# andrewjong/SwapNet

Hardware: NVIDIA H100
Metric: images/sec (G+D fwd+bwd) warp-stage 512x512 (higher is better)
Workload: dtype fp16/bf16-split x3 tensor-core products, fp32 accumulate (fp32-faithful)

## Files before the change

### swapnet_b200/csrc/common.cuh

```cuda
#pragma once
#include <cuda_runtime.h>
#include <cuda.h>
#include <cuda_bf16.h>
#include <cuda_fp16.h>
#include <stdint.h>
#include <stdio.h>
#include <string.h>

void sn_set_error(const char* fmt, ...);
#define SN_OK 0
#define SN_ERR_INVALID (-1)
#define SN_ERR_CUDA (-2)
#define SN_ERR_UNSUPPORTED (-3)
#define SN_NUM_SMS 132
#ifndef SN_FMT_BF16
#define SN_FMT_BF16 0
#define SN_FMT_F16 1
#endif

#define SN_CHECK_CUDA(expr)                                                        \
  do {                                                                             \
    cudaError_t _e = (expr);                                                       \
    if (_e != cudaSuccess) {                                                       \
      sn_set_error("%s:%d CUDA error %s: %s", __FILE__, __LINE__, #expr,           \
// ... 80 lines not shown
      "cp.async.bulk.tensor.3d.shared::cluster.global.mbarrier::complete_tx::bytes"
      " [%0], [%1, {%3, %4, %5}], [%2];"
      :
      : "r"(smem_u32(dst)), "l"(reinterpret_cast<uint64_t>(desc)), "r"(smem_u32(bar)), "r"(c0), "r"(c1), "r"(c2)
      : "memory");
}
__device__ __forceinline__ void tma_load_5d(const void* desc, uint64_t* bar, void* dst, int c0,
                                            int c1, int c2, int c3, int c4) {
  asm volatile(
      "cp.async.bulk.tensor.5d.shared::cluster.global.mbarrier::complete_tx::bytes"
      " [%0], [%1, {%3, %4, %5, %6, %7}], [%2];"
      :
      : "r"(smem_u32(dst)), "l"(reinterpret_cast<uint64_t>(desc)), "r"(smem_u32(bar)), "r"(c0),
        "r"(c1), "r"(c2), "r"(c3), "r"(c4)
      : "memory");
}

__device__ __forceinline__ void wgmma_fence() { asm volatile("wgmma.fence.sync.aligned;" ::: "memory"); }
__device__ __forceinline__ void wgmma_commit() { asm volatile("wgmma.commit_group.sync.aligned;" ::: "memory"); }
template <int N>
__device__ __forceinline__ void wgmma_wait() {
  asm volatile("wgmma.wait_group.sync.aligned %0;" ::"n"(N) : "memory");
}
template <int R>
__device__ __forceinline__ void wgmma_fence_acc(float (&d)[R]) {
#pragma unroll
  for (int i = 0; i < R; ++i) asm volatile("" : "+f"(d[i])::"memory");
}

template <int N, bool F16>
struct Wgmma;
template <> struct Wgmma<16, false> {
  template <int TA, int TB>
  static __device__ __forceinline__ void mma(float (&d)[8], uint64_t a, uint64_t b, int scale_d) {
    asm volatile(
        "{\n.reg .pred p;\nsetp.ne.b32 p, %10, 0;\n"
        "wgmma.mma_async.sync.aligned.m64n16k16.f32.bf16.bf16 "
        "{%0, %1, %2, %3, %4, %5, %6, %7}, %8, %9, p, 1, 1, %11, %12;\n}\n"
        : "+f"(d[0]), "+f"(d[1]), "+f"(d[2]), "+f"(d[3]), "+f"(d[4]), "+f"(d[5]), "+f"(d[6]), "+f"(d[7])
        : "l"(a), "l"(b), "r"(scale_d), "n"(TA), "n"(TB));
  }
};
template <> struct Wgmma<16, true> {
  template <int TA, int TB>
  static __device__ __forceinline__ void mma(float (&d)[8], uint64_t a, uint64_t b, int scale_d) {
    asm volatile(
// ... 72 lines not shown
};
template <> struct Wgmma<128, false> {
  template <int TA, int TB>
  static __device__ __forceinline__ void mma(float (&d)[64], uint64_t a, uint64_t b, int scale_d) {
    asm volatile(
        "{\n.reg .pred p;\nsetp.ne.b32 p, %66, 0;\n"
        "wgmma.mma_async.sync.aligned.m64n128k16.f32.bf16.bf16 "
        "{%0, %1, %2, %3, %4, %5, %6, %7, %8, %9, %10, %11, %12, %13, %14, %15, %16, %17, %18, %19, %20, %21, %22, %23, %24, %25, %26, %27, %28, %29, %30, %31, %32, %33, %34, %35, %36, %37, %38, %39, %40, %41, %42, %43, %44, %45, %46, %47, %48, %49, %50, %51, %52, %53, %54, %55, %56, %57, %58, %59, %60, %61, %62, %63}, %64, %65, p, 1, 1, %67, %68;\n}\n"
        : "+f"(d[0]), "+f"(d[1]), "+f"(d[2]), "+f"(d[3]), "+f"(d[4]), "+f"(d[5]), "+f"(d[6]), "+f"(d[7]), "+f"(d[8]), "+f"(d[9]), "+f"(d[10]), "+f"(d[11]), "+f"(d[12]), "+f"(d[13]), "+f"(d[14]), "+f"(d[15]), "+f"(d[16]), "+f"(d[17]), "+f"(d[18]), "+f"(d[19]), "+f"(d[20]), "+f"(d[21]), "+f"(d[22]), "+f"(d[23]), "+f"(d[24]), "+f"(d[25]), "+f"(d[26]), "+f"(d[27]), "+f"(d[28]), "+f"(d[29]), "+f"(d[30]), "+f"(d[31]), "+f"(d[32]), "+f"(d[33]), "+f"(d[34]), "+f"(d[35]), "+f"(d[36]), "+f"(d[37]), "+f"(d[38]), "+f"(d[39]), "+f"(d[40]), "+f"(d[41]), "+f"(d[42]), "+f"(d[43]), "+f"(d[44]), "+f"(d[45]), "+f"(d[46]), "+f"(d[47]), "+f"(d[48]), "+f"(d[49]), "+f"(d[50]), "+f"(d[51]), "+f"(d[52]), "+f"(d[53]), "+f"(d[54]), "+f"(d[55]), "+f"(d[56]), "+f"(d[57]), "+f"(d[58]), "+f"(d[59]), "+f"(d[60]), "+f"(d[61]), "+f"(d[62]), "+f"(d[63])
        : "l"(a), "l"(b), "r"(scale_d), "n"(TA), "n"(TB));
  }
};
template <> struct Wgmma<128, true> {
  template <int TA, int TB>
  static __device__ __forceinline__ void mma(float (&d)[64], uint64_t a, uint64_t b, int scale_d) {
    asm volatile(
        "{\n.reg .pred p;\nsetp.ne.b32 p, %66, 0;\n"
        "wgmma.mma_async.sync.aligned.m64n128k16.f32.f16.f16 "
        "{%0, %1, %2, %3, %4, %5, %6, %7, %8, %9, %10, %11, %12, %13, %14, %15, %16, %17, %18, %19, %20, %21, %22, %23, %24, %25, %26, %27, %28, %29, %30, %31, %32, %33, %34, %35, %36, %37, %38, %39, %40, %41, %42, %43, %44, %45, %46, %47, %48, %49, %50, %51, %52, %53, %54, %55, %56, %57, %58, %59, %60, %61, %62, %63}, %64, %65, p, 1, 1, %67, %68;\n}\n"
        : "+f"(d[0]), "+f"(d[1]), "+f"(d[2]), "+f"(d[3]), "+f"(d[4]), "+f"(d[5]), "+f"(d[6]), "+f"(d[7]), "+f"(d[8]), "+f"(d[9]), "+f"(d[10]), "+f"(d[11]), "+f"(d[12]), "+f"(d[13]), "+f"(d[14]), "+f"(d[15]), "+f"(d[16]), "+f"(d[17]), "+f"(d[18]), "+f"(d[19]), "+f"(d[20]), "+f"(d[21]), "+f"(d[22]), "+f"(d[23]), "+f"(d[24]), "+f"(d[25]), "+f"(d[26]), "+f"(d[27]), "+f"(d[28]), "+f"(d[29]), "+f"(d[30]), "+f"(d[31]), "+f"(d[32]), "+f"(d[33]), "+f"(d[34]), "+f"(d[35]), "+f"(d[36]), "+f"(d[37]), "+f"(d[38]), "+f"(d[39]), "+f"(d[40]), "+f"(d[41]), "+f"(d[42]), "+f"(d[43]), "+f"(d[44]), "+f"(d[45]), "+f"(d[46]), "+f"(d[47]), "+f"(d[48]), "+f"(d[49]), "+f"(d[50]), "+f"(d[51]), "+f"(d[52]), "+f"(d[53]), "+f"(d[54]), "+f"(d[55]), "+f"(d[56]), "+f"(d[57]), "+f"(d[58]), "+f"(d[59]), "+f"(d[60]), "+f"(d[61]), "+f"(d[62]), "+f"(d[63])
        : "l"(a), "l"(b), "r"(scale_d), "n"(TA), "n"(TB));
  }
};


__device__ __forceinline__ uint64_t gmma_smem_desc(uint32_t smem_addr, uint32_t lbo_bytes, uint32_t sbo_bytes,
                                                   uint32_t layout = 1) {
  uint64_t d = 0;
  d |= (uint64_t)((smem_addr >> 4) & 0x3FFF);
  d |= (uint64_t)((lbo_bytes >> 4) & 0x3FFF) << 16;
  d |= (uint64_t)((sbo_bytes >> 4) & 0x3FFF) << 32;
  d |= (uint64_t)(layout & 3u) << 62;
  return d;
}
__host__ __device__ __forceinline__ uint32_t gmma_layout_of_chunk(int chunk) {
  return chunk >= 64 ? 1u : (chunk == 32 ? 2u : 3u);
}

__device__ __forceinline__ void split16(float v, int fmt, uint16_t& hi, uint16_t& lo) {
  if (fmt == SN_FMT_F16) {
    if (fabsf(v) <= 3.402823466e38f) v = fminf(fmaxf(v, -65504.f), 65504.f);
    const __half h = __float2half_rn(v);
    const __half l = __float2half_rn(v - __half2float(h));
    hi = __half_as_ushort(h);
    lo = __half_as_ushort(l);
  } else {
    const __nv_bfloat16 h = __float2bfloat16_rn(v);
// ... 17 lines not shown
```

### swapnet_b200/csrc/gemm_tc.cu

```cuda
#include "common.cuh"
#include "plan.h"

namespace {

constexpr int kBlockM = 128;
constexpr int kTileRing = 4;
constexpr int kTileBytes = 16384;
constexpr int kConsumerWarps = 8;
constexpr int kProducerWarp = kConsumerWarps;
constexpr int kThreads = (kConsumerWarps + 1) * 32;

template <int NSPLIT>
struct Cfg {
  static constexpr int kPlanes = NSPLIT == 3 ? 2 : 1;
  static constexpr int kStages = NSPLIT == 3 ? 3 : 6;
  static constexpr int kStageBytes = kPlanes * 2 * kTileBytes;
  static constexpr int kSmemBytes = kStages * kStageBytes + 1024;
};

__device__ __forceinline__ float apply_act(float v, int act) {
  if (act == SN_ACT_TANH) return tanhf(v);
  return v;
}

__device__ __forceinline__ float quad_col_sum(float v) {
  v += __shfl_xor_sync(0xffffffffu, v, 4);
  v += __shfl_xor_sync(0xffffffffu, v, 8);
  v += __shfl_xor_sync(0xffffffffu, v, 16);
  return v;
}

template <int NSPLIT, int CW, int BN, bool F16>
__global__ void __launch_bounds__(kThreads, 1)
tap_gemm_kernel(const __grid_constant__ TapGemmParams p, const int m_tiles, const int n_tiles, const int total_tiles) {
  const auto tile_coords = [&](int tile, int& mt, int& nt, int& z) {
    nt = tile % n_tiles;
    const int rest = tile / n_tiles;
    mt = rest % m_tiles;
    z = rest / m_tiles;
  };
  using C = Cfg<NSPLIT>;
  extern __shared__ uint8_t smem_raw[];
  __shared__ __align__(8) uint64_t full_bar[C::kStages];
  __shared__ __align__(8) uint64_t empty_bar[C::kStages];
  __shared__ __align__(8) uint64_t tr_full[kTileRing];
  __shared__ __align__(8) uint64_t tr_empty[kTileRing];
  __shared__ int tile_ring[kTileRing];

  const uint32_t smem_base = (smem_u32(smem_raw) + 1023u) & ~1023u;
  uint8_t* smem = smem_raw + (smem_base - smem_u32(smem_raw));
  const int warp = threadIdx.x >> 5;
  const int lane = threadIdx.x & 31;

  constexpr int cw = CW;
  constexpr int tps = 64 / cw;
  const int tpp = p.ntaps / p.nphase;
  const int k_iters = cw == 64 ? tpp * p.chunks : tpp / tps;

  if (threadIdx.x == 0) {
    for (int s = 0; s < C::kStages; ++s) {
      mbar_init(&full_bar[s], 1);
      mbar_init(&empty_bar[s], 2);
    }
    for (int r = 0; r < kTileRing; ++r) {
      mbar_init(&tr_full[r], 1);
      mbar_init(&tr_empty[r], kConsumerWarps);
    }
    mbar_fence_init();
  }
  if (warp == kProducerWarp && lane == 0) {
    for (int pl = 0; pl < C::kPlanes; ++pl) {
      tma_prefetch_desc(&p.tmA[pl]);
      tma_prefetch_desc(&p.tmB[pl]);
    }
  }
  __syncthreads();

  if (warp == kProducerWarp) {
    if (lane == 0) {
      const uint32_t stage_tx = C::kPlanes * (p.a_rows * 128 + p.block_n * 128);
      uint32_t it = 0, tcount = 0;
      for (int tile = blockIdx.x;; ++tcount) {
        const int next = tile < total_tiles ? (int)gridDim.x + atomicAdd(p.tile_counter, 1) : total_tiles;
        const uint32_t slot = tcount % kTileRing, rph = (tcount / kTileRing) & 1;
        mbar_wait(&tr_empty[slot], rph ^ 1);
        tile_ring[slot] = tile < total_tiles ? tile : -1;
        mbar_arrive(&tr_full[slot]);
        if (tile >= total_tiles) break;
        int mt, nt, z;
        tile_coords(tile, mt, nt, z);
        const int ncol0 = nt * p.block_n;
        const int tap0 = z * tpp;
        const int w0 = (mt % p.tiles_w) * p.tw;
        const int h0 = ((mt / p.tiles_w) % p.tiles_h) * p.th;
        const int n0 = (mt / (p.tiles_w * p.tiles_h)) * p.nb;
        for (int k = 0; k < k_iters; ++k, ++it) {
          const uint32_t s = it % C::kStages;
          const uint32_t ph = (it / C::kStages) & 1;
          mbar_wait(&empty_bar[s], ph ^ 1);
          mbar_expect_tx(&full_bar[s], stage_tx);
          uint8_t* st = smem + s * C::kStageBytes;
          if (cw == 64) {
            const int t = k / p.chunks;
            const int ch = k - t * p.chunks;
            const TapDesc tap = p.taps[tap0 + t];
            if (p.a_merged) {
              tma_load_5d(&p.tmA[0], &full_bar[s], st, tap.c_off + ch * 64, w0 + tap.dw, h0 + tap.dh, n0, 0);
            } else {
#pragma unroll
              for (int pl = 0; pl < C::kPlanes; ++pl)
                tma_load_5d(&p.tmA[pl], &full_bar[s], st + pl * kTileBytes, tap.c_off + ch * 64,
                            w0 + tap.dw, tap.hp, h0 + tap.dh, n0);
            }
            if (p.b_merged) {
              tma_load_3d(&p.tmB[0], &full_bar[s], st + C::kPlanes * kTileBytes, tap.kb_off + ch * 64, ncol0, 0);
            } else {
#pragma unroll
              for (int pl = 0; pl < C::kPlanes; ++pl)
                tma_load_2d(&p.tmB[pl], &full_bar[s], st + (C::kPlanes + pl) * kTileBytes,
                            tap.kb_off + ch * 64, ncol0);
            }
          } else {
            constexpr int sub = 128 * cw * 2;
#pragma unroll
            for (int j = 0; j < tps; ++j) {
              const TapDesc tap = p.taps[tap0 + k * tps + j];
#pragma unroll
              for (int pl = 0; pl < C::kPlanes; ++pl)
                tma_load_5d(&p.tmA[pl], &full_bar[s], st + pl * kTileBytes + j * sub, tap.c_off,
                            w0 + tap.dw, tap.hp, h0 + tap.dh, n0);
            }
            const int kb = p.taps[tap0 + k * tps].kb_off;
            if (p.b_merged) {
              tma_load_3d(&p.tmB[0], &full_bar[s], st + C::kPlanes * kTileBytes, kb, ncol0, 0);
            } else {
#pragma unroll
              for (int pl = 0; pl < C::kPlanes; ++pl)
                tma_load_2d(&p.tmB[pl], &full_bar[s], st + (C::kPlanes + pl) * kTileBytes, kb, ncol0);
            }
          }
        }
        tile = next;
      }
    }
  } else {
    const int wg = warp >> 2;
    const int quad = lane & 3;
    const int row0 = wg * 64 + (warp & 3) * 16 + (lane >> 2);
    int w_i[2], h_i[2], n_i[2];
#pragma unroll
    for (int h = 0; h < 2; ++h) {
      const int row = row0 + 8 * h;
      w_i[h] = row % p.tw;
      h_i[h] = (row / p.tw) % p.th;
      n_i[h] = row / (p.tw * p.th);
    }
    const float oscale = p.b_scale ? p.b_scale[1] : 1.f;
    float acc[BN / 2];
    uint32_t it = 0;
    for (uint32_t tcount = 0;; ++tcount) {
      const uint32_t slot = tcount % kTileRing, rph = (tcount / kTileRing) & 1;
      mbar_wait(&tr_full[slot], rph);
      const int tile = tile_ring[slot];
      __syncwarp();
      if (lane == 0) mbar_arrive(&tr_empty[slot]);
      if (tile < 0) break;
      for (int k = 0; k < k_iters; ++k, ++it) {
        const uint32_t s = it % C::kStages;
        const uint32_t ph = (it / C::kStages) & 1;
        mbar_wait(&full_bar[s], ph);
        const uint32_t st = smem_base + s * C::kStageBytes;
        constexpr uint32_t a_layout = cw >= 64 ? 1u : (cw == 32 ? 2u : 3u);
        constexpr uint32_t a_sbo = 8u * cw * 2u;
        const uint32_t a_row0 = (uint32_t)wg * 64u * cw * 2u;
        const uint64_t a_hi = gmma_smem_desc(st + a_row0, 16, a_sbo, a_layout);
        const uint64_t b_hi = gmma_smem_desc(st + C::kPlanes * kTileBytes, 16, 1024);
        const uint64_t a_lo = gmma_smem_desc(st + p.a_lo_off + a_row0, 16, a_sbo, a_layout);
        const uint64_t b_lo = gmma_smem_desc(st + C::kPlanes * kTileBytes + p.b_lo_off, 16, 1024);
        constexpr uint32_t sub16 = (uint32_t)(128 * cw * 2) >> 4;
        wgmma_fence();
#pragma unroll
        for (int kk = 0; kk < 4; ++kk) {
          const uint64_t badv = (uint64_t)(kk * 2);
          const uint64_t aadv = (uint64_t)(((kk * 16) / cw) * sub16 + (((kk * 16) % cw) >> 3));
          Wgmma<BN, F16>::template mma<0, 0>(acc, a_hi + aadv, b_hi + badv, (k | kk) != 0);
          if (NSPLIT == 3) {
            Wgmma<BN, F16>::template mma<0, 0>(acc, a_lo + aadv, b_hi + badv, 1);
            Wgmma<BN, F16>::template mma<0, 0>(acc, a_hi + aadv, b_lo + badv, 1);
          }
        }
        wgmma_commit();
        wgmma_wait<0>();
        wgmma_fence_acc(acc);
        if ((threadIdx.x & 127) == 0) mbar_arrive(&empty_bar[s]);
      }

      int mt, nt, z;
      tile_coords(tile, mt, nt, z);
      const int ncol0 = nt * p.block_n;
      const int ph_h = p.nphase == 4 ? (z >> 1) : 0, ph_w = p.nphase == 4 ? (z & 1) : 0;
      int gw[2], gh[2], gn[2];
      bool valid[2];
      float* optr[2];
#pragma unroll
      for (int h = 0; h < 2; ++h) {
        gw[h] = (mt % p.tiles_w) * p.tw + w_i[h];
        gh[h] = ((mt / p.tiles_w) % p.tiles_h) * p.th + h_i[h];
// ... 64 lines not shown
              if (col < p.n_valid) optr[h][c] = apply_act(p.bias ? v0 + p.bias[col] : v0, p.act);
              if (col + 1 < p.n_valid) optr[h][c + 1] = apply_act(p.bias ? v1 + p.bias[col + 1] : v1, p.act);
            }
          }
        }
      }
    }
  }

  __syncthreads();
  if (threadIdx.x == 0) {
    __threadfence();
    if (atomicAdd(p.tile_counter + 1, 1) == (int)gridDim.x - 1) {
      p.tile_counter[0] = 0;
      p.tile_counter[1] = 0;
      __threadfence();
    }
  }
}

template <int NSPLIT, int BN, bool F16>
__global__ void __launch_bounds__(kThreads, 1)
wgrad_gemm_kernel(const __grid_constant__ WgradParams p) {
  using C = Cfg<NSPLIT>;
  extern __shared__ uint8_t smem_raw[];
  __shared__ __align__(8) uint64_t full_bar[C::kStages];
  __shared__ __align__(8) uint64_t empty_bar[C::kStages];

  const uint32_t smem_base = (smem_u32(smem_raw) + 1023u) & ~1023u;
  uint8_t* smem = smem_raw + (smem_base - smem_u32(smem_raw));
  const int warp = threadIdx.x >> 5;
  const int lane = threadIdx.x & 31;

  const int m_tile = blockIdx.x / p.n_tiles;
  const int n_tile = blockIdx.x - m_tile * p.n_tiles;
  const bool grouped = p.ngroups > 0;
  const int tap_i = grouped ? p.gstart[blockIdx.y] : blockIdx.y;
  const int gsize = grouped ? p.gsize[blockIdx.y] : 1;
  const int m0 = m_tile * kBlockM;
  const int ncol0 = n_tile * p.block_n;
  const int total = p.tiles_w * p.tiles_h * p.tiles_n;
  const int kt0 = (int)(((long long)total * blockIdx.z) / gridDim.z);
  const int kt1 = (int)(((long long)total * (blockIdx.z + 1)) / gridDim.z);
  const int k_iters = kt1 - kt0;
  const int ycw = p.y_chunk;
  const int y_blocks = ycw == 64 ? p.block_n / 64 : gsize;
  const int y_block_bytes = 64 * ycw * 2;
// ... 178 lines not shown
    strides[3] = (cuuint64_t)H * W * pitch * e;
  } else {
    SN_REQUIRE(H % 2 == 0 && W % 2 == 0, "parity view needs even H, W (got %d x %d)", H, W);
    dims[0] = (cuuint64_t)pitch + C; dims[1] = W / 2; dims[2] = 2; dims[3] = H / 2; dims[4] = N;
    strides[0] = (cuuint64_t)2 * pitch * e;
    strides[1] = (cuuint64_t)W * pitch * e;
    strides[2] = (cuuint64_t)2 * W * pitch * e;
    strides[3] = (cuuint64_t)H * W * pitch * e;
  }
  SN_REQUIRE(chunk == 64 || chunk == 32 || chunk == 16, "row chunk must be 64, 32 or 16 channels (got %d)", chunk);
  cuuint32_t estr[5] = {1, 1, 1, 1, 1};
  const CUtensorMapSwizzle swz = chunk == 64 ? CU_TENSOR_MAP_SWIZZLE_128B
                                 : chunk == 32 ? CU_TENSOR_MAP_SWIZZLE_64B : CU_TENSOR_MAP_SWIZZLE_32B;
  CUresult r = enc(tm, CU_TENSOR_MAP_DATA_TYPE_BFLOAT16, 5, const_cast<void*>(base), dims, strides,
                   box, estr, CU_TENSOR_MAP_INTERLEAVE_NONE, swz,
                   CU_TENSOR_MAP_L2_PROMOTION_L2_256B, CU_TENSOR_MAP_FLOAT_OOB_FILL_NONE);
  SN_REQUIRE(r == CUDA_SUCCESS,
             "cuTensorMapEncodeTiled(act) failed: %d (N=%d H=%d W=%d C=%d pitch=%d parity=%d box=%dx%dx%d)",
             (int)r, N, H, W, C, pitch, parity, box_w, box_h, box_n);
  return SN_OK;
}

int sn_make_weight_map(CUtensorMap* tm, const void* base, int rows, long long k_total, int box_rows,
                       long long plane_stride = 0) {
  PFN_encodeTiled enc = get_encode_fn();
  SN_REQUIRE(enc != nullptr, "cuTensorMapEncodeTiled driver entry point unavailable");
  SN_REQUIRE(k_total % 64 == 0 && ((uintptr_t)base % 16) == 0, "packed weights need K %% 64 == 0");
  cuuint64_t dims[3] = {(cuuint64_t)k_total, (cuuint64_t)rows, 2};
  cuuint64_t strides[2] = {(cuuint64_t)k_total * 2, (cuuint64_t)plane_stride};
  cuuint32_t box[3] = {64, (cuuint32_t)box_rows, 2};
  cuuint32_t estr[3] = {1, 1, 1};
  CUresult r = enc(tm, CU_TENSOR_MAP_DATA_TYPE_BFLOAT16, plane_stride > 0 ? 3 : 2, const_cast<void*>(base), dims, strides,
                   box, estr, CU_TENSOR_MAP_INTERLEAVE_NONE, CU_TENSOR_MAP_SWIZZLE_128B,
                   CU_TENSOR_MAP_L2_PROMOTION_L2_256B, CU_TENSOR_MAP_FLOAT_OOB_FILL_NONE);
  SN_REQUIRE(r == CUDA_SUCCESS, "cuTensorMapEncodeTiled(weights) failed: %d (rows=%d K=%lld box_rows=%d)",
             (int)r, rows, k_total, box_rows);
  return SN_OK;
}

static void pick_patch(int m_h, int m_w, int rows, int* th, int* tw, int* nb) {
  int w = 16;
  while (w > 1 && w / 2 >= m_w) w /= 2;
  if (w > rows) w = rows;
  int h = rows / w;
  while (h > 1 && h / 2 >= m_h) h /= 2;
  *tw = w;
  *th = h;
  *nb = rows / (w * h);
}

static void pick_patch_conv(int m_n, int m_h, int m_w, int* th, int* tw, int* nb) {
  double best_eff = -1.0;
  int best_perim = 1 << 30, best_rows = 0, best_area = 0;
  const long long useful = (long long)m_n * m_h * m_w;
  for (int w = 1; w <= m_w && w <= 128; ++w) {
    for (int h = 1; h <= m_h && h * w <= 128; ++h) {
// ... 15 lines not shown
      if (better) {
        best_eff = eff; best_rows = rows; best_perim = perim; best_area = area;
        *tw = w; *th = h; *nb = n;
      }
    }
  }
}

int sn_tap_gemm_plan_init(TapGemmPlan* plan, const sn_tap_gemm_desc* d) {
  memset(plan, 0, sizeof(*plan));
  TapGemmParams& p = plan->p;
  SN_REQUIRE(d->nsplit == 1 || d->nsplit == 3, "nsplit must be 1 or 3");
  SN_REQUIRE(d->ntaps >= 1 && d->ntaps <= SN_MAX_TAPS, "ntaps out of range: %d", d->ntaps);
  const int a_chunk = d->a_chunk ? d->a_chunk : 64;
  SN_REQUIRE(a_chunk == 64 || a_chunk == 32 || a_chunk == 16, "a_chunk must be 64, 32 or 16");
  if (a_chunk == 64) {
    SN_REQUIRE(d->k_per_tap > 0 && d->k_per_tap % 64 == 0, "k_per_tap must be a multiple of 64");
  } else {
    SN_REQUIRE(d->k_per_tap == a_chunk && d->ntaps % (64 / a_chunk) == 0,
               "narrow operand: k_per_tap must equal a_chunk (%d) and ntaps (%d) be a multiple of %d", a_chunk,
               d->ntaps, 64 / a_chunk);
  }
  p.a_chunk = a_chunk;
  SN_REQUIRE(d->block_n >= 16 && d->block_n <= 128 && d->block_n % 16 == 0,
             "block_n must be a multiple of 16 in [16,128]");
  SN_REQUIRE(d->a_hi && d->b_hi && d->out, "null operand");
  SN_REQUIRE(d->nsplit == 1 || (d->a_lo && d->b_lo), "nsplit=3 needs lo planes");
  SN_REQUIRE(d->a_fmt == d->b_fmt, "A and B of one wgmma must share a 16-bit format (a=%d b=%d)",
             d->a_fmt, d->b_fmt);
  int th, tw, nb;
  pick_patch_conv(d->m_n, d->m_h, d->m_w, &th, &tw, &nb);
  p.a_rows = th * tw * nb;
  p.tw = tw; p.th = th; p.nb = nb;
  p.tiles_w = (d->m_w + tw - 1) / tw;
  p.tiles_h = (d->m_h + th - 1) / th;
  p.tiles_n = (d->m_n + nb - 1) / nb;
  p.m_w = d->m_w; p.m_h = d->m_h; p.m_n = d->m_n;
  p.ntaps = d->ntaps;
  p.chunks = a_chunk == 64 ? d->k_per_tap / 64 : 1;
  for (int t = 0; t < d->ntaps; ++t) {
    p.taps[t].c_off = d->taps[t].c_off;
    p.taps[t].kb_off = d->taps[t].kb_off;
    p.taps[t].dw = (short)d->taps[t].dw;
    p.taps[t].dh = (short)d->taps[t].dh;
    p.taps[t].hp = (short)d->taps[t].hp;
  }
  p.block_n = d->block_n;
  p.n_valid = d->n_valid;
// ... 16 lines not shown
               "phase-stacked output: n_valid = 4*stack_slot, nphase 1, out_mul 2 (slot=%d c=%d n_valid=%d)",
               d->stack_slot, d->stack_c, d->n_valid);
  p.b_scale = d->b_scale;
  p.a_fmt = d->a_fmt;
  p.b_fmt = d->b_fmt;
  p.act = d->act;
  p.vec4 = ((uintptr_t)d->out % 16 == 0) && (d->out_sn % 4 == 0) && (d->out_sh % 4 == 0) &&
           (d->out_sw % 4 == 0) && (!d->bias || (uintptr_t)d->bias % 16 == 0);
  if (d->stats && nb == 1 && p.vec4 && d->n_valid % 16 == 0 && d->act == 0 && d->stack_slot == 0 && d->m_n * 1 >= 1)
    p.stats = d->stats;
  plan->stats_bytes = p.stats ? sizeof(double) * 2 * (size_t)d->m_n * d->n_valid : 0;
  p.tile_counter = nullptr;
  SN_CHECK_CUDA(cudaMalloc(&p.tile_counter, 2 * sizeof(int)));
  SN_CHECK_CUDA(cudaMemset(p.tile_counter, 0, 2 * sizeof(int)));
  int rc;
  const void* a_pl[2] = {d->a_hi, d->a_lo};
  const void* b_pl[2] = {d->b_hi, d->b_lo};
  const long long a_ps = d->nsplit == 3 ? (const char*)d->a_lo - (const char*)d->a_hi : 0;
  const long long b_ps = d->nsplit == 3 ? (const char*)d->b_lo - (const char*)d->b_hi : 0;
  p.a_merged = a_chunk == 64 && a_ps > 0 && a_ps % 16 == 0 && p.a_rows % 8 == 0;
  if (p.a_merged && d->a_parity)
    for (int t = 0; t < d->ntaps; ++t) p.taps[t].c_off += p.taps[t].hp * d->a_w * d->a_pitch;
  p.b_merged = b_ps > 0 && b_ps % 16 == 0 && d->block_n % 8 == 0;
  p.a_lo_off = p.a_merged ? p.a_rows * 128 : kTileBytes;
  p.b_lo_off = p.b_merged ? d->block_n * 128 : kTileBytes;
  for (int pl = 0; pl < (d->nsplit == 3 ? 2 : 1); ++pl) {
    if (!(p.a_merged && pl == 1)) {
      rc = sn_make_act_map(&p.tmA[pl], a_pl[pl], d->a_n, d->a_h, d->a_w, d->a_c, d->a_pitch,
                           d->a_parity, tw, th, nb, a_chunk, p.a_merged ? a_ps : 0);
      if (rc) return rc;
    }
    if (!(p.b_merged && pl == 1)) {
      rc = sn_make_weight_map(&p.tmB[pl], b_pl[pl], d->b_rows, d->b_k, d->block_n, p.b_merged ? b_ps : 0);
      if (rc) return rc;
    }
  }
  if (p.a_merged) p.tmA[1] = p.tmA[0];
  if (p.b_merged) p.tmB[1] = p.tmB[0];
  plan->nsplit = d->nsplit;
  plan->grid = dim3(p.tiles_w * p.tiles_h * p.tiles_n, (d->n_valid + d->block_n - 1) / d->block_n, p.nphase);
  return SN_OK;
}

static int mma_n(int block_n) {
  return block_n <= 16 ? 16 : block_n <= 32 ? 32 : block_n <= 64 ? 64 : block_n <= 96 ? 96 : 128;
}

template <int NSPLIT, int CW, int BN, bool F16>
static int launch_tap(const TapGemmPlan* plan, cudaStream_t stream) {
  static bool attr_done = false;
  if (!attr_done) {
    SN_CHECK_CUDA(cudaFuncSetAttribute(tap_gemm_kernel<NSPLIT, CW, BN, F16>, cudaFuncAttributeMaxDynamicSharedMemorySize,
                                       Cfg<NSPLIT>::kSmemBytes));
    attr_done = true;
  }
  static int sms = 0;
  if (sms == 0) {
    int dev = 0;
    SN_CHECK_CUDA(cudaGetDevice(&dev));
    SN_CHECK_CUDA(cudaDeviceGetAttribute(&sms, cudaDevAttrMultiProcessorCount, dev));
  }
  const int m_tiles = (int)plan->grid.x, n_tiles = (int)plan->grid.y;
  const int total = m_tiles * n_tiles * (int)plan->grid.z;
  if (plan->p.stats) SN_CHECK_CUDA(cudaMemsetAsync(plan->p.stats, 0, plan->stats_bytes, stream));
  const int ctas = total < sms ? total : sms;
  tap_gemm_kernel<NSPLIT, CW, BN, F16>
      <<<ctas, kThreads, Cfg<NSPLIT>::kSmemBytes, stream>>>(plan->p, m_tiles, n_tiles, total);
  SN_CHECK_CUDA(cudaGetLastError());
  return SN_OK;
}

template <int NSPLIT, int CW, bool F16>
static int launch_tap_n(const TapGemmPlan* plan, cudaStream_t stream) {
  switch (mma_n(plan->p.block_n)) {
    case 16: return launch_tap<NSPLIT, CW, 16, F16>(plan, stream);
    case 32: return launch_tap<NSPLIT, CW, 32, F16>(plan, stream);
    case 64: return launch_tap<NSPLIT, CW, 64, F16>(plan, stream);
    case 96: return launch_tap<NSPLIT, CW, 96, F16>(plan, stream);
    default: return launch_tap<NSPLIT, CW, 128, F16>(plan, stream);
  }
}

template <int NSPLIT, bool F16>
static int launch_tap_cw(const TapGemmPlan* plan, cudaStream_t stream) {
  const int cw = plan->p.a_chunk;
  if (cw == 64) return launch_tap_n<NSPLIT, 64, F16>(plan, stream);
  if (cw == 32) return launch_tap_n<NSPLIT, 32, F16>(plan, stream);
  return launch_tap_n<NSPLIT, 16, F16>(plan, stream);
}

int sn_tap_gemm_plan_launch(const TapGemmPlan* plan, cudaStream_t stream) {
  const bool f16 = plan->p.a_fmt == SN_FMT_F16;
  if (plan->nsplit == 3) return f16 ? launch_tap_cw<3, true>(plan, stream) : launch_tap_cw<3, false>(plan, stream);
  return f16 ? launch_tap_cw<1, true>(plan, stream) : launch_tap_cw<1, false>(plan, stream);
}

int sn_wgrad_plan_init(WgradPlan* plan, const sn_wgrad_desc* d, int sm_count) {
  memset(plan, 0, sizeof(*plan));
  WgradParams& p = plan->p;
  SN_REQUIRE(d->nsplit == 1 || d->nsplit == 3, "nsplit must be 1 or 3");
  SN_REQUIRE(d->ntaps >= 1 && d->ntaps <= SN_MAX_TAPS, "ntaps out of range: %d", d->ntaps);
  const int y_chunk = d->y_chunk ? d->y_chunk : 64;
// ... 79 lines not shown
    if (p.y_merged) p.tmY[1] = p.tmY[0];
  }
  plan->nsplit = d->nsplit;
  const int base_ctas = p.m_tiles * p.n_tiles * grid_y;
  const int total = p.tiles_w * p.tiles_h * p.tiles_n;
  int ks = d->ksplit;
  if (ks <= 0) {
    ks = (3 * sm_count + base_ctas - 1) / base_ctas;
    int max_ks = total / 8;
    if (max_ks < 1) max_ks = 1;
    if (ks > max_ks) ks = max_ks;
    if (ks < 1) ks = 1;
  }
  if (ks > total) ks = total;
  plan->grid = dim3(p.m_tiles * p.n_tiles, grid_y, ks);
  return SN_OK;
}

template <int NSPLIT, int BN, bool F16>
static int launch_wgrad(const WgradPlan* plan, cudaStream_t stream) {
  static bool attr_done = false;
  if (!attr_done) {
    SN_CHECK_CUDA(cudaFuncSetAttribute(wgrad_gemm_kernel<NSPLIT, BN, F16>, cudaFuncAttributeMaxDynamicSharedMemorySize,
                                       Cfg<NSPLIT>::kSmemBytes));
    attr_done = true;
  }
  wgrad_gemm_kernel<NSPLIT, BN, F16><<<plan->grid, kThreads, Cfg<NSPLIT>::kSmemBytes, stream>>>(plan->p);
  SN_CHECK_CUDA(cudaGetLastError());
  return SN_OK;
}

template <int NSPLIT, bool F16>
static int launch_wgrad_n(const WgradPlan* plan, cudaStream_t stream) {
  switch (mma_n(plan->p.block_n)) {
    case 16: return launch_wgrad<NSPLIT, 16, F16>(plan, stream);
    case 32: return launch_wgrad<NSPLIT, 32, F16>(plan, stream);
    case 64: return launch_wgrad<NSPLIT, 64, F16>(plan, stream);
    case 96: return launch_wgrad<NSPLIT, 96, F16>(plan, stream);
    default: return launch_wgrad<NSPLIT, 128, F16>(plan, stream);
  }
}

int sn_wgrad_plan_launch(const WgradPlan* plan, cudaStream_t stream) {
  const bool f16 = plan->p.x_fmt == SN_FMT_F16;
  if (plan->nsplit == 3) return f16 ? launch_wgrad_n<3, true>(plan, stream) : launch_wgrad_n<3, false>(plan, stream);
  return f16 ? launch_wgrad_n<1, true>(plan, stream) : launch_wgrad_n<1, false>(plan, stream);
}
```

### swapnet_b200/layers.py

```python
from __future__ import annotations

from typing import List, Optional

import torch

from . import lowering as L
from . import ops
from .ops import ACT_NONE, PackedWeights, Planes


class ConvLayer:
    def __init__(self, kind: str, weight: torch.Tensor, bias: Optional[torch.Tensor], x: Planes, *,
                 nsplit: int = 3, act: int = ACT_NONE, name: str = ""):
        assert kind in L.KINDS
        self.kind, self.name, self.nsplit, self.act = kind, name, nsplit, act
        self.weight, self.bias = weight, bias
        self.x = x
        dev = weight.device
        if kind == "convT4s2":
            self.cin, self.cout = weight.shape[0], weight.shape[1]
        else:
            self.cout, self.cin = weight.shape[0], weight.shape[1]
        self.in_h, self.in_w = (x.h - 2, x.w - 2) if kind == "conv3r" else (x.h, x.w)
        self.out_h, self.out_w = L.out_hw(kind, self.in_h, self.in_w)
        self.n = x.n
        self.k_pad = x.c
        assert (self.k_pad % 64 == 0 or self.k_pad in (16, 32)) and self.k_pad >= self.cin, (name, x.c, self.cin)
        self.block_n = L.pick_block_n(self.cout)
        self.t = L.ntaps(kind)
        self.wscale = torch.ones(2, dtype=torch.float32, device=dev)
        self.stacked = kind == "head" and self.cout <= L.HEAD_SLOT and self.k_pad % 64 == 0
        if self.stacked:
            self.rows_pad = 4 * L.HEAD_SLOT
            self.wp = PackedWeights(self.rows_pad, 9 * self.k_pad, dev, self.wscale)
        elif kind == "head":
            self.rows_pad = (self.cout + self.block_n - 1) // self.block_n * self.block_n
            self.wp = PackedWeights(self.rows_pad, 25 * self.k_pad, dev, self.wscale)
        else:
            self.wp = PackedWeights(self.cout, self._tpad(self.t, self.k_pad) * self.k_pad, dev, self.wscale)
        self.fwd_plans: List[ops.Plan] = []
        self.y: Optional[torch.Tensor] = None
        self.wd: Optional[PackedWeights] = None
        self.dy: Optional[Planes] = None
        self.dgrad_plans: List[ops.Plan] = []
        self.wgrad_plan: Optional[ops.Plan] = None
        self.dx: Optional[torch.Tensor] = None
        self.wgrad_out: Optional[torch.Tensor] = None
        self.bgrad_out: Optional[torch.Tensor] = None
        self._geff: Optional[torch.Tensor] = None
        self._bscratch: Optional[torch.Tensor] = None

# ... 206 lines not shown
```

### swapnet_b200/lowering.py

```python
from __future__ import annotations

from dataclasses import dataclass, field
from typing import List, Tuple

KINDS = ("conv4s2", "convT4s2", "conv3r", "conv4s1", "head", "conv3z")

@dataclass
class Tap:
    pw: int
    kb: int
    dw: int
    dh: int
    hp: int = 0


@dataclass
class GemmSpec:
    parity: bool
    m_h: int
    m_w: int
    taps: List[Tap]
    out_mul: Tuple[int, int] = (1, 1)
    out_off: Tuple[int, int] = (0, 0)
    w_phase: int = 0
# ... 198 lines not shown
def wgrad_out_strides(kind: str, cin: int, cout: int, x_is_dy: bool) -> Tuple[int, int]:
    t = ntaps(kind)
    if kind == "head":
        co_s, ci_s = 25 * cin, 1
    elif kind == "convT4s2":
        ci_s, co_s = cout * t, t
    else:
        co_s, ci_s = cin * t, t
    return (co_s, ci_s) if x_is_dy else (ci_s, co_s)


def pad64(c: int) -> int:
    return (c + 63) // 64 * 64


def padc(c: int) -> int:
    if c <= 16:
        return 16
    if c <= 32:
        return 32
    return pad64(c)


def pick_block_n(n_valid: int) -> int:
    if n_valid >= 128:
        return 128
    for b in (16, 32, 64, 128):
        if n_valid <= b:
            return b
    return 128
```

Measured before the change: 102.9.

## Add 256-column wgmma tile path for wide split-precision tap GEMMs

Adds an m64n256k16 wgmma variant and a BN=256 configuration of the tap GEMM kernel. It uses 32-deep K slices with 64B swizzle, a 4-stage ring and 384 threads, and uses setmaxnreg to move registers from the producer warps to the consumers. Layers with nsplit 3, 64-channel rows, cout a multiple of 256 and at least 512, and enough tiles now pick this wider tile. The goal is better operand reuse per A load and fewer B reloads. The trade-off is heavy register pressure, halved K per stage, and fewer tiles to spread across SMs.

```diff
diff --git a/swapnet_b200/csrc/common.cuh b/swapnet_b200/csrc/common.cuh
--- a/swapnet_b200/csrc/common.cuh
+++ b/swapnet_b200/csrc/common.cuh
@@ -126,6 +126,10 @@
 __device__ __forceinline__ void wgmma_wait() {
   asm volatile("wgmma.wait_group.sync.aligned %0;" ::"n"(N) : "memory");
 }
+template <int N>
+__device__ __forceinline__ void warpgroup_reg_alloc() { asm volatile("setmaxnreg.inc.sync.aligned.u32 %0;" ::"n"(N)); }
+template <int N>
+__device__ __forceinline__ void warpgroup_reg_dealloc() { asm volatile("setmaxnreg.dec.sync.aligned.u32 %0;" ::"n"(N)); }
 template <int R>
 __device__ __forceinline__ void wgmma_fence_acc(float (&d)[R]) {
 #pragma unroll
@@ -244,7 +248,28 @@
         : "l"(a), "l"(b), "r"(scale_d), "n"(TA), "n"(TB));
   }
 };
-
+template <> struct Wgmma<256, false> {
+  template <int TA, int TB>
+  static __device__ __forceinline__ void mma(float (&d)[128], uint64_t a, uint64_t b, int scale_d) {
+    asm volatile(
+        "{\n.reg .pred p;\nsetp.ne.b32 p, %130, 0;\n"
+        "wgmma.mma_async.sync.aligned.m64n256k16.f32.bf16.bf16 "
+        "{%0, %1, %2, %3, %4, %5, %6, %7, %8, %9, %10, %11, %12, %13, %14, %15, %16, %17, %18, %19, %20, %21, %22, %23, %24, %25, %26, %27, %28, %29, %30, %31, %32, %33, %34, %35, %36, %37, %38, %39, %40, %41, %42, %43, %44, %45, %46, %47, %48, %49, %50, %51, %52, %53, %54, %55, %56, %57, %58, %59, %60, %61, %62, %63, %64, %65, %66, %67, %68, %69, %70, %71, %72, %73, %74, %75, %76, %77, %78, %79, %80, %81, %82, %83, %84, %85, %86, %87, %88, %89, %90, %91, %92, %93, %94, %95, %96, %97, %98, %99, %100, %101, %102, %103, %104, %105, %106, %107, %108, %109, %110, %111, %112, %113, %114, %115, %116, %117, %118, %119, %120, %121, %122, %123, %124, %125, %126, %127}, %128, %129, p, 1, 1, %131, %132;\n}\n"
+        : "+f"(d[0]), "+f"(d[1]), "+f"(d[2]), "+f"(d[3]), "+f"(d[4]), "+f"(d[5]), "+f"(d[6]), "+f"(d[7]), "+f"(d[8]), "+f"(d[9]), "+f"(d[10]), "+f"(d[11]), "+f"(d[12]), "+f"(d[13]), "+f"(d[14]), "+f"(d[15]), "+f"(d[16]), "+f"(d[17]), "+f"(d[18]), "+f"(d[19]), "+f"(d[20]), "+f"(d[21]), "+f"(d[22]), "+f"(d[23]), "+f"(d[24]), "+f"(d[25]), "+f"(d[26]), "+f"(d[27]), "+f"(d[28]), "+f"(d[29]), "+f"(d[30]), "+f"(d[31]), "+f"(d[32]), "+f"(d[33]), "+f"(d[34]), "+f"(d[35]), "+f"(d[36]), "+f"(d[37]), "+f"(d[38]), "+f"(d[39]), "+f"(d[40]), "+f"(d[41]), "+f"(d[42]), "+f"(d[43]), "+f"(d[44]), "+f"(d[45]), "+f"(d[46]), "+f"(d[47]), "+f"(d[48]), "+f"(d[49]), "+f"(d[50]), "+f"(d[51]), "+f"(d[52]), "+f"(d[53]), "+f"(d[54]), "+f"(d[55]), "+f"(d[56]), "+f"(d[57]), "+f"(d[58]), "+f"(d[59]), "+f"(d[60]), "+f"(d[61]), "+f"(d[62]), "+f"(d[63]), "+f"(d[64]), "+f"(d[65]), "+f"(d[66]), "+f"(d[67]), "+f"(d[68]), "+f"(d[69]), "+f"(d[70]), "+f"(d[71]), "+f"(d[72]), "+f"(d[73]), "+f"(d[74]), "+f"(d[75]), "+f"(d[76]), "+f"(d[77]), "+f"(d[78]), "+f"(d[79]), "+f"(d[80]), "+f"(d[81]), "+f"(d[82]), "+f"(d[83]), "+f"(d[84]), "+f"(d[85]), "+f"(d[86]), "+f"(d[87]), "+f"(d[88]), "+f"(d[89]), "+f"(d[90]), "+f"(d[91]), "+f"(d[92]), "+f"(d[93]), "+f"(d[94]), "+f"(d[95]), "+f"(d[96]), "+f"(d[97]), "+f"(d[98]), "+f"(d[99]), "+f"(d[100]), "+f"(d[101]), "+f"(d[102]), "+f"(d[103]), "+f"(d[104]), "+f"(d[105]), "+f"(d[106]), "+f"(d[107]), "+f"(d[108]), "+f"(d[109]), "+f"(d[110]), "+f"(d[111]), "+f"(d[112]), "+f"(d[113]), "+f"(d[114]), "+f"(d[115]), "+f"(d[116]), "+f"(d[117]), "+f"(d[118]), "+f"(d[119]), "+f"(d[120]), "+f"(d[121]), "+f"(d[122]), "+f"(d[123]), "+f"(d[124]), "+f"(d[125]), "+f"(d[126]), "+f"(d[127])
+        : "l"(a), "l"(b), "r"(scale_d), "n"(TA), "n"(TB));
+  }
+};
+template <> struct Wgmma<256, true> {
+  template <int TA, int TB>
+  static __device__ __forceinline__ void mma(float (&d)[128], uint64_t a, uint64_t b, int scale_d) {
+    asm volatile(
+        "{\n.reg .pred p;\nsetp.ne.b32 p, %130, 0;\n"
+        "wgmma.mma_async.sync.aligned.m64n256k16.f32.f16.f16 "
+        "{%0, %1, %2, %3, %4, %5, %6, %7, %8, %9, %10, %11, %12, %13, %14, %15, %16, %17, %18, %19, %20, %21, %22, %23, %24, %25, %26, %27, %28, %29, %30, %31, %32, %33, %34, %35, %36, %37, %38, %39, %40, %41, %42, %43, %44, %45, %46, %47, %48, %49, %50, %51, %52, %53, %54, %55, %56, %57, %58, %59, %60, %61, %62, %63, %64, %65, %66, %67, %68, %69, %70, %71, %72, %73, %74, %75, %76, %77, %78, %79, %80, %81, %82, %83, %84, %85, %86, %87, %88, %89, %90, %91, %92, %93, %94, %95, %96, %97, %98, %99, %100, %101, %102, %103, %104, %105, %106, %107, %108, %109, %110, %111, %112, %113, %114, %115, %116, %117, %118, %119, %120, %121, %122, %123, %124, %125, %126, %127}, %128, %129, p, 1, 1, %131, %132;\n}\n"
+        : "+f"(d[0]), "+f"(d[1]), "+f"(d[2]), "+f"(d[3]), "+f"(d[4]), "+f"(d[5]), "+f"(d[6]), "+f"(d[7]), "+f"(d[8]), "+f"(d[9]), "+f"(d[10]), "+f"(d[11]), "+f"(d[12]), "+f"(d[13]), "+f"(d[14]), "+f"(d[15]), "+f"(d[16]), "+f"(d[17]), "+f"(d[18]), "+f"(d[19]), "+f"(d[20]), "+f"(d[21]), "+f"(d[22]), "+f"(d[23]), "+f"(d[24]), "+f"(d[25]), "+f"(d[26]), "+f"(d[27]), "+f"(d[28]), "+f"(d[29]), "+f"(d[30]), "+f"(d[31]), "+f"(d[32]), "+f"(d[33]), "+f"(d[34]), "+f"(d[35]), "+f"(d[36]), "+f"(d[37]), "+f"(d[38]), "+f"(d[39]), "+f"(d[40]), "+f"(d[41]), "+f"(d[42]), "+f"(d[43]), "+f"(d[44]), "+f"(d[45]), "+f"(d[46]), "+f"(d[47]), "+f"(d[48]), "+f"(d[49]), "+f"(d[50]), "+f"(d[51]), "+f"(d[52]), "+f"(d[53]), "+f"(d[54]), "+f"(d[55]), "+f"(d[56]), "+f"(d[57]), "+f"(d[58]), "+f"(d[59]), "+f"(d[60]), "+f"(d[61]), "+f"(d[62]), "+f"(d[63]), "+f"(d[64]), "+f"(d[65]), "+f"(d[66]), "+f"(d[67]), "+f"(d[68]), "+f"(d[69]), "+f"(d[70]), "+f"(d[71]), "+f"(d[72]), "+f"(d[73]), "+f"(d[74]), "+f"(d[75]), "+f"(d[76]), "+f"(d[77]), "+f"(d[78]), "+f"(d[79]), "+f"(d[80]), "+f"(d[81]), "+f"(d[82]), "+f"(d[83]), "+f"(d[84]), "+f"(d[85]), "+f"(d[86]), "+f"(d[87]), "+f"(d[88]), "+f"(d[89]), "+f"(d[90]), "+f"(d[91]), "+f"(d[92]), "+f"(d[93]), "+f"(d[94]), "+f"(d[95]), "+f"(d[96]), "+f"(d[97]), "+f"(d[98]), "+f"(d[99]), "+f"(d[100]), "+f"(d[101]), "+f"(d[102]), "+f"(d[103]), "+f"(d[104]), "+f"(d[105]), "+f"(d[106]), "+f"(d[107]), "+f"(d[108]), "+f"(d[109]), "+f"(d[110]), "+f"(d[111]), "+f"(d[112]), "+f"(d[113]), "+f"(d[114]), "+f"(d[115]), "+f"(d[116]), "+f"(d[117]), "+f"(d[118]), "+f"(d[119]), "+f"(d[120]), "+f"(d[121]), "+f"(d[122]), "+f"(d[123]), "+f"(d[124]), "+f"(d[125]), "+f"(d[126]), "+f"(d[127])
+        : "l"(a), "l"(b), "r"(scale_d), "n"(TA), "n"(TB));
+  }
+};
 
 __device__ __forceinline__ uint64_t gmma_smem_desc(uint32_t smem_addr, uint32_t lbo_bytes, uint32_t sbo_bytes,
                                                    uint32_t layout = 1) {
diff --git a/swapnet_b200/csrc/gemm_tc.cu b/swapnet_b200/csrc/gemm_tc.cu
--- a/swapnet_b200/csrc/gemm_tc.cu
+++ b/swapnet_b200/csrc/gemm_tc.cu
@@ -10,11 +10,15 @@
 constexpr int kProducerWarp = kConsumerWarps;
 constexpr int kThreads = (kConsumerWarps + 1) * 32;
 
-template <int NSPLIT>
+template <int NSPLIT, int BN>
 struct Cfg {
   static constexpr int kPlanes = NSPLIT == 3 ? 2 : 1;
-  static constexpr int kStages = NSPLIT == 3 ? 3 : 6;
-  static constexpr int kStageBytes = kPlanes * 2 * kTileBytes;
+  static constexpr int kK = BN == 256 ? 32 : 64;
+  static constexpr int kRowBytes = kK * 2;
+  static constexpr int kATile = kBlockM * kRowBytes;
+  static constexpr int kBTile = (BN == 256 ? 256 : 128) * kRowBytes;
+  static constexpr int kStages = BN == 256 ? 4 : (NSPLIT == 3 ? 3 : 6);
+  static constexpr int kStageBytes = kPlanes * (kATile + kBTile);
   static constexpr int kSmemBytes = kStages * kStageBytes + 1024;
 };
 
@@ -30,8 +34,11 @@
   return v;
 }
 
+template <int BN>
+constexpr int tap_threads() { return BN == 256 ? 384 : kThreads; }
+
 template <int NSPLIT, int CW, int BN, bool F16>
-__global__ void __launch_bounds__(kThreads, 1)
+__global__ void __launch_bounds__(tap_threads<BN>(), 1)
 tap_gemm_kernel(const __grid_constant__ TapGemmParams p, const int m_tiles, const int n_tiles, const int total_tiles) {
   const auto tile_coords = [&](int tile, int& mt, int& nt, int& z) {
     nt = tile % n_tiles;
@@ -39,7 +46,8 @@
     mt = rest % m_tiles;
     z = rest / m_tiles;
   };
-  using C = Cfg<NSPLIT>;
+  using C = Cfg<NSPLIT, BN>;
+  static_assert(BN <= 128 || (NSPLIT == 3 && CW == 64), "256-column tiles: split operands with 64-channel rows only");
   extern __shared__ uint8_t smem_raw[];
   __shared__ __align__(8) uint64_t full_bar[C::kStages];
   __shared__ __align__(8) uint64_t empty_bar[C::kStages];
@@ -54,8 +62,10 @@
 
   constexpr int cw = CW;
   constexpr int tps = 64 / cw;
+  constexpr int spc = 64 / C::kK;
+  constexpr int aw = cw == 64 ? C::kK : cw;
   const int tpp = p.ntaps / p.nphase;
-  const int k_iters = cw == 64 ? tpp * p.chunks : tpp / tps;
+  const int k_iters = cw == 64 ? tpp * p.chunks * spc : tpp / tps;
 
   if (threadIdx.x == 0) {
     for (int s = 0; s < C::kStages; ++s) {
@@ -76,9 +86,10 @@
   }
   __syncthreads();
 
-  if (warp == kProducerWarp) {
-    if (lane == 0) {
-      const uint32_t stage_tx = C::kPlanes * (p.a_rows * 128 + p.block_n * 128);
+  if (warp >= kProducerWarp) {
+    if constexpr (BN == 256) warpgroup_reg_dealloc<40>();
+    if (warp == kProducerWarp && lane == 0) {
+      const uint32_t stage_tx = C::kPlanes * (p.a_rows + p.block_n) * C::kRowBytes;
       uint32_t it = 0, tcount = 0;
       for (int tile = blockIdx.x;; ++tcount) {
         const int next = tile < total_tiles ? (int)gridDim.x + atomicAdd(p.tile_counter, 1) : total_tiles;
@@ -101,24 +112,26 @@
           mbar_expect_tx(&full_bar[s], stage_tx);
           uint8_t* st = smem + s * C::kStageBytes;
           if (cw == 64) {
-            const int t = k / p.chunks;
-            const int ch = k - t * p.chunks;
+            const int kc = k / spc;
+            const int t = kc / p.chunks;
+            const int ch = kc - t * p.chunks;
+            const int kcol = ch * 64 + (k - kc * spc) * C::kK;
             const TapDesc tap = p.taps[tap0 + t];
             if (p.a_merged) {
-              tma_load_5d(&p.tmA[0], &full_bar[s], st, tap.c_off + ch * 64, w0 + tap.dw, h0 + tap.dh, n0, 0);
+              tma_load_5d(&p.tmA[0], &full_bar[s], st, tap.c_off + kcol, w0 + tap.dw, h0 + tap.dh, n0, 0);
             } else {
 #pragma unroll
               for (int pl = 0; pl < C::kPlanes; ++pl)
-                tma_load_5d(&p.tmA[pl], &full_bar[s], st + pl * kTileBytes, tap.c_off + ch * 64,
+                tma_load_5d(&p.tmA[pl], &full_bar[s], st + pl * C::kATile, tap.c_off + kcol,
                             w0 + tap.dw, tap.hp, h0 + tap.dh, n0);
             }
             if (p.b_merged) {
-              tma_load_3d(&p.tmB[0], &full_bar[s], st + C::kPlanes * kTileBytes, tap.kb_off + ch * 64, ncol0, 0);
+              tma_load_3d(&p.tmB[0], &full_bar[s], st + C::kPlanes * C::kATile, tap.kb_off + kcol, ncol0, 0);
             } else {
 #pragma unroll
               for (int pl = 0; pl < C::kPlanes; ++pl)
-                tma_load_2d(&p.tmB[pl], &full_bar[s], st + (C::kPlanes + pl) * kTileBytes,
-                            tap.kb_off + ch * 64, ncol0);
+                tma_load_2d(&p.tmB[pl], &full_bar[s], st + C::kPlanes * C::kATile + pl * C::kBTile,
+                            tap.kb_off + kcol, ncol0);
             }
           } else {
             constexpr int sub = 128 * cw * 2;
@@ -127,16 +140,16 @@
               const TapDesc tap = p.taps[tap0 + k * tps + j];
 #pragma unroll
               for (int pl = 0; pl < C::kPlanes; ++pl)
-                tma_load_5d(&p.tmA[pl], &full_bar[s], st + pl * kTileBytes + j * sub, tap.c_off,
+                tma_load_5d(&p.tmA[pl], &full_bar[s], st + pl * C::kATile + j * sub, tap.c_off,
                             w0 + tap.dw, tap.hp, h0 + tap.dh, n0);
             }
             const int kb = p.taps[tap0 + k * tps].kb_off;
             if (p.b_merged) {
-              tma_load_3d(&p.tmB[0], &full_bar[s], st + C::kPlanes * kTileBytes, kb, ncol0, 0);
+              tma_load_3d(&p.tmB[0], &full_bar[s], st + C::kPlanes * C::kATile, kb, ncol0, 0);
             } else {
 #pragma unroll
               for (int pl = 0; pl < C::kPlanes; ++pl)
-                tma_load_2d(&p.tmB[pl], &full_bar[s], st + (C::kPlanes + pl) * kTileBytes, kb, ncol0);
+                tma_load_2d(&p.tmB[pl], &full_bar[s], st + C::kPlanes * C::kATile + pl * C::kBTile, kb, ncol0);
             }
           }
         }
@@ -144,6 +157,7 @@
       }
     }
   } else {
+    if constexpr (BN == 256) warpgroup_reg_alloc<232>();
     const int wg = warp >> 2;
     const int quad = lane & 3;
     const int row0 = wg * 64 + (warp & 3) * 16 + (lane >> 2);
@@ -170,19 +184,21 @@
         const uint32_t ph = (it / C::kStages) & 1;
         mbar_wait(&full_bar[s], ph);
         const uint32_t st = smem_base + s * C::kStageBytes;
-        constexpr uint32_t a_layout = cw >= 64 ? 1u : (cw == 32 ? 2u : 3u);
-        constexpr uint32_t a_sbo = 8u * cw * 2u;
-        const uint32_t a_row0 = (uint32_t)wg * 64u * cw * 2u;
+        constexpr uint32_t a_layout = aw >= 64 ? 1u : (aw == 32 ? 2u : 3u);
+        constexpr uint32_t a_sbo = 8u * aw * 2u;
+        constexpr uint32_t b_layout = C::kK == 64 ? 1u : 2u;
+        constexpr uint32_t b_sbo = 8u * C::kRowBytes;
+        const uint32_t a_row0 = (uint32_t)wg * 64u * aw * 2u;
         const uint64_t a_hi = gmma_smem_desc(st + a_row0, 16, a_sbo, a_layout);
-        const uint64_t b_hi = gmma_smem_desc(st + C::kPlanes * kTileBytes, 16, 1024);
+        const uint64_t b_hi = gmma_smem_desc(st + C::kPlanes * C::kATile, 16, b_sbo, b_layout);
         const uint64_t a_lo = gmma_smem_desc(st + p.a_lo_off + a_row0, 16, a_sbo, a_layout);
-        const uint64_t b_lo = gmma_smem_desc(st + C::kPlanes * kTileBytes + p.b_lo_off, 16, 1024);
-        constexpr uint32_t sub16 = (uint32_t)(128 * cw * 2) >> 4;
+        const uint64_t b_lo = gmma_smem_desc(st + C::kPlanes * C::kATile + p.b_lo_off, 16, b_sbo, b_layout);
+        constexpr uint32_t sub16 = (uint32_t)(128 * aw * 2) >> 4;
         wgmma_fence();
 #pragma unroll
-        for (int kk = 0; kk < 4; ++kk) {
+        for (int kk = 0; kk < C::kK / 16; ++kk) {
           const uint64_t badv = (uint64_t)(kk * 2);
-          const uint64_t aadv = (uint64_t)(((kk * 16) / cw) * sub16 + (((kk * 16) % cw) >> 3));
+          const uint64_t aadv = (uint64_t)(((kk * 16) / aw) * sub16 + (((kk * 16) % aw) >> 3));
           Wgmma<BN, F16>::template mma<0, 0>(acc, a_hi + aadv, b_hi + badv, (k | kk) != 0);
           if (NSPLIT == 3) {
             Wgmma<BN, F16>::template mma<0, 0>(acc, a_lo + aadv, b_hi + badv, 1);
@@ -293,7 +309,7 @@
 template <int NSPLIT, int BN, bool F16>
 __global__ void __launch_bounds__(kThreads, 1)
 wgrad_gemm_kernel(const __grid_constant__ WgradParams p) {
-  using C = Cfg<NSPLIT>;
+  using C = Cfg<NSPLIT, BN>;
   extern __shared__ uint8_t smem_raw[];
   __shared__ __align__(8) uint64_t full_bar[C::kStages];
   __shared__ __align__(8) uint64_t empty_bar[C::kStages];
@@ -518,16 +534,18 @@
 }
 
 int sn_make_weight_map(CUtensorMap* tm, const void* base, int rows, long long k_total, int box_rows,
-                       long long plane_stride = 0) {
+                       long long plane_stride = 0, int box_k = 64) {
   PFN_encodeTiled enc = get_encode_fn();
   SN_REQUIRE(enc != nullptr, "cuTensorMapEncodeTiled driver entry point unavailable");
   SN_REQUIRE(k_total % 64 == 0 && ((uintptr_t)base % 16) == 0, "packed weights need K %% 64 == 0");
+  SN_REQUIRE(box_k == 64 || box_k == 32, "weight box depth must be 64 or 32 (got %d)", box_k);
   cuuint64_t dims[3] = {(cuuint64_t)k_total, (cuuint64_t)rows, 2};
   cuuint64_t strides[2] = {(cuuint64_t)k_total * 2, (cuuint64_t)plane_stride};
-  cuuint32_t box[3] = {64, (cuuint32_t)box_rows, 2};
+  cuuint32_t box[3] = {(cuuint32_t)box_k, (cuuint32_t)box_rows, 2};
   cuuint32_t estr[3] = {1, 1, 1};
   CUresult r = enc(tm, CU_TENSOR_MAP_DATA_TYPE_BFLOAT16, plane_stride > 0 ? 3 : 2, const_cast<void*>(base), dims, strides,
-                   box, estr, CU_TENSOR_MAP_INTERLEAVE_NONE, CU_TENSOR_MAP_SWIZZLE_128B,
+                   box, estr, CU_TENSOR_MAP_INTERLEAVE_NONE,
+                   box_k == 64 ? CU_TENSOR_MAP_SWIZZLE_128B : CU_TENSOR_MAP_SWIZZLE_64B,
                    CU_TENSOR_MAP_L2_PROMOTION_L2_256B, CU_TENSOR_MAP_FLOAT_OOB_FILL_NONE);
   SN_REQUIRE(r == CUDA_SUCCESS, "cuTensorMapEncodeTiled(weights) failed: %d (rows=%d K=%lld box_rows=%d)",
              (int)r, rows, k_total, box_rows);
@@ -589,8 +607,12 @@
                d->ntaps, 64 / a_chunk);
   }
   p.a_chunk = a_chunk;
-  SN_REQUIRE(d->block_n >= 16 && d->block_n <= 128 && d->block_n % 16 == 0,
-             "block_n must be a multiple of 16 in [16,128]");
+  SN_REQUIRE((d->block_n >= 16 && d->block_n <= 128 && d->block_n % 16 == 0) ||
+                 (d->block_n == 256 && d->nsplit == 3 && a_chunk == 64),
+             "block_n must be a multiple of 16 in [16,128], or 256 for nsplit 3 with 64-channel A rows (got %d)",
+             d->block_n);
+  const int wide = d->block_n == 256;
+  const int row_bytes = wide ? 64 : 128;
   SN_REQUIRE(d->a_hi && d->b_hi && d->out, "null operand");
   SN_REQUIRE(d->nsplit == 1 || (d->a_lo && d->b_lo), "nsplit=3 needs lo planes");
   SN_REQUIRE(d->a_fmt == d->b_fmt, "A and B of one wgmma must share a 16-bit format (a=%d b=%d)",
@@ -653,16 +675,17 @@
   if (p.a_merged && d->a_parity)
     for (int t = 0; t < d->ntaps; ++t) p.taps[t].c_off += p.taps[t].hp * d->a_w * d->a_pitch;
   p.b_merged = b_ps > 0 && b_ps % 16 == 0 && d->block_n % 8 == 0;
-  p.a_lo_off = p.a_merged ? p.a_rows * 128 : kTileBytes;
-  p.b_lo_off = p.b_merged ? d->block_n * 128 : kTileBytes;
+  p.a_lo_off = p.a_merged ? p.a_rows * row_bytes : kBlockM * row_bytes;
+  p.b_lo_off = p.b_merged ? d->block_n * row_bytes : kTileBytes;
   for (int pl = 0; pl < (d->nsplit == 3 ? 2 : 1); ++pl) {
     if (!(p.a_merged && pl == 1)) {
       rc = sn_make_act_map(&p.tmA[pl], a_pl[pl], d->a_n, d->a_h, d->a_w, d->a_c, d->a_pitch,
-                           d->a_parity, tw, th, nb, a_chunk, p.a_merged ? a_ps : 0);
+                           d->a_parity, tw, th, nb, wide ? 32 : a_chunk, p.a_merged ? a_ps : 0);
       if (rc) return rc;
     }
     if (!(p.b_merged && pl == 1)) {
-      rc = sn_make_weight_map(&p.tmB[pl], b_pl[pl], d->b_rows, d->b_k, d->block_n, p.b_merged ? b_ps : 0);
+      rc = sn_make_weight_map(&p.tmB[pl], b_pl[pl], d->b_rows, d->b_k, d->block_n, p.b_merged ? b_ps : 0,
+                              wide ? 32 : 64);
       if (rc) return rc;
     }
   }
@@ -674,7 +697,7 @@
 }
 
 static int mma_n(int block_n) {
-  return block_n <= 16 ? 16 : block_n <= 32 ? 32 : block_n <= 64 ? 64 : block_n <= 96 ? 96 : 128;
+  return block_n <= 16 ? 16 : block_n <= 32 ? 32 : block_n <= 64 ? 64 : block_n <= 96 ? 96 : block_n <= 128 ? 128 : 256;
 }
 
 template <int NSPLIT, int CW, int BN, bool F16>
@@ -682,7 +705,7 @@
   static bool attr_done = false;
   if (!attr_done) {
     SN_CHECK_CUDA(cudaFuncSetAttribute(tap_gemm_kernel<NSPLIT, CW, BN, F16>, cudaFuncAttributeMaxDynamicSharedMemorySize,
-                                       Cfg<NSPLIT>::kSmemBytes));
+                                       Cfg<NSPLIT, BN>::kSmemBytes));
     attr_done = true;
   }
   static int sms = 0;
@@ -696,7 +719,7 @@
   if (plan->p.stats) SN_CHECK_CUDA(cudaMemsetAsync(plan->p.stats, 0, plan->stats_bytes, stream));
   const int ctas = total < sms ? total : sms;
   tap_gemm_kernel<NSPLIT, CW, BN, F16>
-      <<<ctas, kThreads, Cfg<NSPLIT>::kSmemBytes, stream>>>(plan->p, m_tiles, n_tiles, total);
+      <<<ctas, tap_threads<BN>(), Cfg<NSPLIT, BN>::kSmemBytes, stream>>>(plan->p, m_tiles, n_tiles, total);
   SN_CHECK_CUDA(cudaGetLastError());
   return SN_OK;
 }
@@ -708,7 +731,13 @@
     case 32: return launch_tap<NSPLIT, CW, 32, F16>(plan, stream);
     case 64: return launch_tap<NSPLIT, CW, 64, F16>(plan, stream);
     case 96: return launch_tap<NSPLIT, CW, 96, F16>(plan, stream);
-    default: return launch_tap<NSPLIT, CW, 128, F16>(plan, stream);
+    case 128: return launch_tap<NSPLIT, CW, 128, F16>(plan, stream);
+    default:
+      if constexpr (NSPLIT == 3 && CW == 64) {
+        return launch_tap<NSPLIT, CW, 256, F16>(plan, stream);
+      } else {
+        SN_REQUIRE(false, "no 256-column tap GEMM for nsplit %d, %d-channel rows", NSPLIT, CW);
+      }
   }
 }
 
@@ -834,10 +863,10 @@
   static bool attr_done = false;
   if (!attr_done) {
     SN_CHECK_CUDA(cudaFuncSetAttribute(wgrad_gemm_kernel<NSPLIT, BN, F16>, cudaFuncAttributeMaxDynamicSharedMemorySize,
-                                       Cfg<NSPLIT>::kSmemBytes));
+                                       Cfg<NSPLIT, BN>::kSmemBytes));
     attr_done = true;
   }
-  wgrad_gemm_kernel<NSPLIT, BN, F16><<<plan->grid, kThreads, Cfg<NSPLIT>::kSmemBytes, stream>>>(plan->p);
+  wgrad_gemm_kernel<NSPLIT, BN, F16><<<plan->grid, kThreads, Cfg<NSPLIT, BN>::kSmemBytes, stream>>>(plan->p);
   SN_CHECK_CUDA(cudaGetLastError());
   return SN_OK;
 }
diff --git a/swapnet_b200/layers.py b/swapnet_b200/layers.py
--- a/swapnet_b200/layers.py
+++ b/swapnet_b200/layers.py
@@ -26,7 +26,8 @@
         self.n = x.n
         self.k_pad = x.c
         assert (self.k_pad % 64 == 0 or self.k_pad in (16, 32)) and self.k_pad >= self.cin, (name, x.c, self.cin)
-        self.block_n = L.pick_block_n(self.cout)
+        self.block_n = L.pick_block_n(self.cout, wide=nsplit == 3 and self.k_pad % 64 == 0 and kind not in ("convT4s2", "head"),
+                                      m_rows=self.n * self.out_h * self.out_w)
         self.t = L.ntaps(kind)
         self.wscale = torch.ones(2, dtype=torch.float32, device=dev)
         self.stacked = kind == "head" and self.cout <= L.HEAD_SLOT and self.k_pad % 64 == 0
diff --git a/swapnet_b200/lowering.py b/swapnet_b200/lowering.py
--- a/swapnet_b200/lowering.py
+++ b/swapnet_b200/lowering.py
@@ -244,7 +244,12 @@
     return pad64(c)
 
 
-def pick_block_n(n_valid: int) -> int:
+WIDE_MIN_TILES = 2 * 132
+
+
+def pick_block_n(n_valid: int, wide: bool = False, m_rows: int = 0) -> int:
+    if wide and n_valid % 256 == 0 and n_valid >= 512 and -(-m_rows // 128) * (n_valid // 256) >= WIDE_MIN_TILES:
+        return 256
     if n_valid >= 128:
         return 128
     for b in (16, 32, 64, 128):
```

Result: faster. 104.0 (median of 6 runs) (+1.1%).
